# ddiazdom/grlBWT

Measured on AMD Instinct MI355X. Metric: input MB/s building BCR BWT on 10 GB DNA reads, 1/2/4/8 MI355X, higher is better.
Workload: dtype u8; 1 GPU; 66225166 x 150 bp Illumina-style reads (10000000066 bytes) from a 330000000 bp genome, 0.5% substitutions; BASELINE configs[3]; input_resident=HBM, output=.rl_bwt image in HBM, parallelism=1 GPU

## Files before the change

### grlbwt_amd/csrc/engine_impl.hpp

```cpp

#include "switches.hpp"

namespace GRL_NS {

using prim::u8;
using prim::u16;
using prim::u32;
using prim::u64;
typedef GRL_IDX_T idx_t;

template <class T>
struct DBuf {
    T *p = nullptr;
    u64 n = 0;
    DBuf() {}
    explicit DBuf(u64 n_) { alloc(n_); }
    DBuf(const DBuf &) = delete;
    DBuf &operator=(const DBuf &) = delete;
    DBuf(DBuf &&o) noexcept : p(o.p), n(o.n) { o.p = nullptr; o.n = 0; }
    DBuf &operator=(DBuf &&o) noexcept {
        if (this != &o) { release(); p = o.p; n = o.n; o.p = nullptr; o.n = 0; }
        return *this;
    }
    ~DBuf() { release(); }
    void alloc(u64 n_) { release(); p = (T *)prim::dev_alloc((n_ ? n_ : 1) * sizeof(T)); n = n_; }
    void release() { if (p) prim::dev_free(p); p = nullptr; n = 0; }
    void shrink(u64 n_) { if (p && n_ < n) { prim::dev_shrink(p, (n_ ? n_ : 1) * sizeof(T)); n = n_; } }
    void zero() { prim::dev_memset(p, 0, n * sizeof(T)); }
    void fill_ff() { prim::dev_memset(p, 0xFF, n * sizeof(T)); }
    std::vector<T> to_host(u64 cnt) const { std::vector<T> h(cnt); prim::d2h(h.data(), p, cnt * sizeof(T)); return h; }
    T get(u64 i) const { T v; prim::d2h(&v, p + i, sizeof(T)); return v; }
};

static inline unsigned bitlen64(u64 v) { return v == 0 ? 0 : 64 - (unsigned)__builtin_clzll(v); }

static inline bool test_fail_rank(int fail_rank, int me) {
    if constexpr (prim::kIsDevice) { (void)fail_rank; (void)me; return false; }
    else return fail_rank == me;
}

template <class T>
GRL_HD u64 upper_bound(const T *a, u64 n, T v) {
    u64 lo = 0, hi = n;
    while (lo < hi) { u64 mid = (lo + hi) >> 1; if (a[mid] <= v) lo = mid + 1; else hi = mid; }
// ... 639 lines not shown
    }
};
template <class F>
struct ListedFn {
    F f; const u64 *pos;
    static constexpr int kBatch = 1;
    static constexpr bool kClaims = F::kClaims;
    u64 *claim_bits = nullptr;
    GRL_DEV u64 claim_pos(u64 v) const { return pos[v]; }
    GRL_DEV bool is_start(u64) const { return true; }
    GRL_DEV u32 process(u64 v) const { return f.process(pos[v]); }
    GRL_DEV u32 operator()(u64 v) const { return f.process(pos[v]); }
    GRL_DEV void process_batch(const u64 *, const bool *, u32 *) const {}
    GRL_DEV void first_seen(u32 slot, u64 v) const { f.first_seen(slot, pos[v]); }
};

template <class cell_t, bool FIRST>
struct CompactTableFn {
    const cell_t *t;
    CellOps<cell_t, FIRST> ops;
    const u64 *startbits;
    const u64 *keys; const idx_t *counts;
    u64 *ph_pos; idx_t *ph_freq; u32 *ph_len; u32 *ph_slot; u8 *ph_lastT;
    int ks; u64 cs; const u64 *rep_pos;
    u64 n;
    GRL_DEV void emit(u64 s, u64 k) const {
        u64 k64 = keys[s << ks];
        u64 pos, len;
        bool lastT;
        if (k64 & kExactKey) {
// ... 43 lines not shown
        const u64 k0 = pbase[p], cnt = (u64)pbase[p + 1] - k0, src0 = pstart[p];
        for (u64 j = i & 63; j < cnt; j += 64) {
            const u64 k = k0 + j, src = src0 + j;
            const u64 hi = dhi[src];
            const prim::U128 r(rec_lo(dkey[src], hi), hi);
            const u32 f = dcnt[src];
            ph_key[k] = r; ph_pos[k] = 0; ph_freq[k] = (idx_t)f; ph_len[k] = rec_len(r); ph_slot[k] = slot0 + (u32)k;
            ph_lastT[k] = (r.hi & kPhrLastT) ? 1 : 0;
            ph_vflag[k] = (u8)((f > 1 ? 2u : 0u) | ((r.hi & kPhrLastT) ? 1u : 0u));
        }
    }
};
struct PartValFn {
    const u64 *pstart; const u32 *pbase; const u32 *lid; const u32 *slot_val; u32 slot0; u32 *out;
    const u8 *vflag;
    GRL_DEV void operator()(u64 i) const {
        const u64 p = i >> 6;
        const u64 a = pstart[p], e = pstart[p + 1], k0 = (u64)pbase[p], v0 = (u64)slot0 + k0;
        for (u64 x = a + (i & 63); x < e; x += 256) {
            u32 l[4], v[4];
#pragma unroll
            for (int j = 0; j < 4; j++) l[j] = x + 64u * j < e ? lid[x + 64u * j] : prim::kNoId;
#pragma unroll
            for (int j = 0; j < 4; j++) v[j] = l[j] == prim::kNoId ? 0u : (slot_val[v0 + (u64)l[j]] | (vflag ? (u32)vflag[k0 + (u64)l[j]] : 0u));
#pragma unroll
            for (int j = 0; j < 4; j++) if (x + 64u * j < e) out[x + 64u * j] = v[j];
        }
    }
};
struct PartCombineFn {
    const u32 *slot_val; const u32 *vals; u32 *text;
    GRL_DEV void operator()(u64 i) const { const u32 m = text[i]; text[i] = (m & kLongMark) ? slot_val[m & ~kLongMark] : vals[i]; }
};
struct LenIn {
    const u32 *l;
    GRL_DEV u32 operator()(u64 i) const { return l[i]; }
};
struct FreqLenIn {
    const idx_t *f; const u32 *l;
    GRL_DEV prim::Pair<u64, u64> operator()(u64 i) const { return prim::Pair<u64, u64>((u64)f[i], (u64)l[i]); }
};
GRL_HD u64 rank1(const u64 *words, const idx_t *base, u64 x);
template <class cell_t, bool FIRST, int PER = 4>
struct DictBuildFn {
    const cell_t *t;
    CellOps<cell_t, FIRST> ops;
    const u32 *ph_off; u64 D; u64 S; const u64 *ph_pos;
// ... 819 lines not shown
                u64 x = x16[k], w = x >> 6;
                if (w != cur) { prim::atomic_or(&words[cur * ws], m); m = 0; cur = w; }
                m |= 1ull << (x & 63);
            }
        }
        prim::atomic_or(&words[cur * ws], m);
    }
};
GRL_HD u64 rank1(const u64 *words, const idx_t *base, u64 x) {
    return (u64)base[x >> 6] + (u64)__builtin_popcountll(words[x >> 6] & ((1ull << (x & 63)) - 1ull));
}
static inline void build_rankbits(RankBits &rb, const idx_t *pos, u64 count, u64 nbits, const char *name) {
    u64 nw = nbits / 64 + 2;
    rb.words.alloc(nw);
    rb.base.alloc(nw + 1);
    rb.words.zero();
    prim::for_each((count + 15) / 16, BuildBitsFn{pos, count, rb.words.p}, name);
    prim::exclusive_scan_nosync<idx_t>(nw, PopcIn{rb.words.p}, rb.base.p, true, name);
}

struct BuildBits32Fn {
    const u32 *pos; u64 count; u64 *words;
    GRL_DEV void operator()(u64 j) const {
        u64 i0 = j * 16, i1 = i0 + 16 < count ? i0 + 16 : count;
        u64 cur = (u64)pos[i0] >> 6, m = 0;
        for (u64 i = i0; i < i1; i++) {
            u64 x = pos[i], w = x >> 6;
            if (w != cur) { prim::atomic_or(&words[cur], m); m = 0; cur = w; }
            m |= 1ull << (x & 63);
        }
        prim::atomic_or(&words[cur], m);
    }
};
static inline void build_rankbits32(RankBits &rb, const u32 *pos, u64 count, u64 nbits, const char *name) {
    u64 nw = nbits / 64 + 2;
    rb.words.alloc(nw);
    rb.base.alloc(nw + 1);
    rb.words.zero();
    prim::for_each((count + 15) / 16, BuildBits32Fn{pos, count, rb.words.p}, name);
    prim::exclusive_scan_nosync<idx_t>(nw, PopcIn{rb.words.p}, rb.base.p, true, name);
}

template <class L>
struct IdxIn {
    const L *p;
    GRL_DEV idx_t operator()(u64 i) const { return (idx_t)p[i]; }
};
struct SymHeadIn64 {
    const u32 *s;
    GRL_DEV u64 operator()(u64 t) const { return (t == 0 || s[t] != s[t - 1]) ? 1ull : 0ull; }
};
struct IdxIn64 {
    const idx_t *p;
// ... 1083 lines not shown
        prim::h2d(own0.p, host_cells, n * (u64)w);
        load_text(own0.p, n, w);
    }

    struct LocalParse {
        u64 n_occ = 0, D = 0, S = 0, cap = 0;
        u32 maxlen = 0;
        DBuf<u32> next_text;
        DBuf<u64> ph_pos; DBuf<idx_t> ph_freq; DBuf<u32> ph_len, ph_slot, ph_off; DBuf<u8> ph_lastT;
        u64 Ds = 0; int part_bits = 0, rec_b = 0; u32 slot0 = 0;
        DBuf<prim::U128> ph_key;
        DBuf<u32> lid, pbase;
        DBuf<u8> ph_vflag;
        DBuf<u64> pstart;
        prim::RecSort psort;
        void clear() {
            n_occ = D = S = cap = Ds = 0; maxlen = 0; part_bits = rec_b = 0; slot0 = 0;
            next_text.release(); ph_pos.release(); ph_freq.release(); ph_len.release(); ph_slot.release(); ph_off.release(); ph_lastT.release();
            ph_key.release(); ph_vflag.release(); pstart.release(); lid.release(); pbase.release(); psort.release();
        }
    };

    struct PartPlan { bool on = false; int rec_b = 0; u32 rec_cmax = 0; int part_bits = 0; };
    struct SamplePlan { u64 blk = 0, stride = 0, n = 0, distinct = 0, long_occ = 0; double frac = 1.0; };
    struct TablePlan { u64 cap = 0, cap_max = 0, cap_hot = 0; bool aggregate = false, interleaved = false, direct = false; int ks = 0; u64 cs = 1; u32 dir_b[3] = {0, 0, 0}; u64 sym_of_code = 0; };
    static bool direct_index_bits(const u64 sym_present[4], u32 bits[3], u64 &sym_of_code) {
        int syms[256], ns = 0;
        for (int i = 0; i < 256; i++) if ((sym_present[i >> 6] >> (i & 63)) & 1ull) syms[ns++] = i;
        if (ns > 8) return false;
        for (u32 a = 0; a < 8; a++) for (u32 b = a + 1; b < 8; b++) for (u32 c = b + 1; c < 8; c++) {
            u32 seen = 0; bool ok = true; u64 soc = 0;
            for (int k = 0; k < ns && ok; k++) {
// ... 41 lines not shown
            while (part.part_bits < 20 && (n_occ >> part.part_bits) > 5000) part.part_bits++;
            if (prim::sw().part_bits) part.part_bits = std::max(1, std::min(20, prim::sw().part_bits));
        }
        void sample_table() {
            tab.cap_max = 1024;
            while (tab.cap_max < 2 * n_occ && tab.cap_max < (1ull << 31)) tab.cap_max <<= 1;
            tab.cap = tab.cap_max;
            P.next_text.alloc(n_occ); scal.alloc(8); giant_list.alloc(giant_cap);
            StageTimer st(&E.tm.hash, "hash");
            const u64 want_s = (FIRST && n >= (1ull << 26)) ? (1ull << 22) : (1ull << 20), n_s = n < want_s ? n : want_s;
            if (n_s >= n) return;
            smp.blk = 4096; smp.stride = n / (n_s / smp.blk); smp.n = n_s;
            u64 cap_s = 1024; while (cap_s < 2 * n_s) cap_s <<= 1;
            DBuf<u64> tk(cap_s), trep; DBuf<idx_t> tc(cap_s);
            if (HF::kExact) trep.alloc(cap_s);
            tk.zero(); tc.zero(); scal.zero();
            HF fs{t, ops, startbits.p, wordbase.p, tk.p, cap_s - 1, cap_s, 0, P.next_text.p, scal.p, n, n_occ, trep.p};
            fs.rec_b = part.rec_b; fs.rec_cmax = part.rec_cmax;
            fs.walk_cap = HF::kLongWalk;
            prim::for_each_agg(n_s, SampledFn<HF>{fs, smp.blk, smp.stride}, SlotCountAdd{tc.p, 1}, true, "hash_sample");
            const prim::Pair<u64, u64> so = prim::reduce_sum<prim::Pair<u64, u64>>(cap_s, SampleCountIn{tk.p, tc.p}, "hash_sample_count");
            const u64 occ_s = std::max<u64>(so.b, 1);
            smp.distinct = so.a;
            if (part.on) smp.long_occ = occ_s;
            smp.frac = std::min(1.0, (double)smp.distinct / (double)occ_s);
            u64 want = (u64)(1.7 * smp.frac * (double)n_occ) + 4096;
            if (part.on) want = (u64)(3.0 * (double)smp.long_occ * ((double)n / (double)n_s)) + 4096;
            tab.cap = 4096; while (tab.cap < want) tab.cap <<= 1;
            if (tab.cap > tab.cap_max) tab.cap = tab.cap_max;
            if (prim::sw().table_trace) fprintf(stderr, "[grlbwt] level %d: sample %llu occurrences, %llu distinct -> table %llu slots for %llu occurrences\n",
                                                      prim::rt().tag, (unsigned long long)occ_s, (unsigned long long)smp.distinct, (unsigned long long)tab.cap, (unsigned long long)n_occ);
// ... 15 lines not shown
                }
            }
            const bool hot = !tab.direct && tab.aggregate && smp.n && !part.on && !prim::sw().no_hot_table;
            if (!tab.direct && !hot) return;
            if (tab.direct) tab.cap_hot = HF::kDirectSlots;
            else for (tab.cap_hot = 1024; tab.cap_hot < 4 * smp.distinct;) tab.cap_hot <<= 1;
            if (tab.cap_max > (1ull << 30)) tab.cap_max = 1ull << 30;
            if (tab.cap > tab.cap_max) tab.cap = tab.cap_max;
            if (!prim::sw().table_trace) return;
            if (tab.direct) fprintf(stderr, "[grlbwt] level %d: direct index on bits %u, %u, %u of a cell (%llu slots in front of the table)\n", prim::rt().tag,
                                    tab.dir_b[0], tab.dir_b[1], tab.dir_b[2], (unsigned long long)tab.cap_hot);
            else fprintf(stderr, "[grlbwt] level %d: hot table of %llu slots for the %llu phrases of the sample\n", prim::rt().tag,
                         (unsigned long long)tab.cap_hot, (unsigned long long)smp.distinct);
        }
        void alloc_table() {
            if (tab.interleaved) { keys.alloc(2 * tab.cap); keys.zero(); }
            else { keys.alloc(tab.cap_hot + tab.cap); counts.alloc(tab.cap_hot + tab.cap); keys.zero(); counts.zero(); }
            cnt = tab.interleaved ? (idx_t *)(keys.p + 1) : counts.p;
            if (HF::kExact) rep_pos.alloc(tab.cap_hot + tab.cap);
            scal.zero(); claim.zero();
        }
        void fill_hot_table(HF &f) {
            HF fh{t, ops, startbits.p, wordbase.p, keys.p, tab.cap_hot - 1, tab.cap_hot, 0, P.next_text.p, scal.p, n, n_occ, rep_pos.p, claim.p};
            fh.walk_cap = HF::kLongWalk;
            prim::for_each_agg(smp.n, SampledFn<HF>{fh, smp.blk, smp.stride, claim.p}, NoCountAdd{}, false, "hash_hot");
            f.hot_keys = keys.p; f.hot_mask = tab.cap_hot - 1; f.slot_base = (u32)tab.cap_hot;
        }
        void hash_listed(const HF &f, DBuf<u64> &lbits, bool aggregate) {
            DBuf<u32> lbase(nwords + 1);
            const u64 nl = (u64)prim::exclusive_scan<u32>(nwords, PopcIn32{lbits.p}, lbase.p, false, "hash_long_list");
            DBuf<u64> lpos(nl ? nl : 1);
            if (nl) prim::for_each(nwords, BitPositionsFn{lbits.p, lbase.p, lpos.p}, "hash_long_list");
            lbits.release(); lbase.release();
            if (nl) prim::for_each_agg(nl, ListedFn<HF>{f, lpos.p, claim.p}, SlotCountAdd{cnt, tab.cs}, aggregate, "hash_long_phrases");
        }
        void records_and_long_phrases(const HF &f) {
            prim::dev_memset(P.next_text.p, 0, n_occ * sizeof(u32));
            DBuf<u64> lbits(nwords + 1); lbits.zero();
            auto records = [&](auto bw) {
                prim::for_each_set_bit<idx_t>(n, startbits.p, wordbase.p, PhraseRecordFn<cell_t, decltype(bw)::value>{t, ops, startbits.p, wordbase.p, n, n_occ,
                                                                                                               rec_k.p, rec_hi.p, part.rec_b, part.rec_cmax, lbits.p, scal.p}, "hash_phrases");
            };
            switch (part.rec_b) {
#define GRL_REC_CASE(BW) case BW: records(std::integral_constant<int, BW>()); break;
                GRL_REC_CASE(10) GRL_REC_CASE(11) GRL_REC_CASE(12) GRL_REC_CASE(13) GRL_REC_CASE(14) GRL_REC_CASE(15) GRL_REC_CASE(16)
                GRL_REC_CASE(17) GRL_REC_CASE(18) GRL_REC_CASE(19) GRL_REC_CASE(20) GRL_REC_CASE(21) GRL_REC_CASE(22) GRL_REC_CASE(23)
                GRL_REC_CASE(24) GRL_REC_CASE(25) GRL_REC_CASE(26) GRL_REC_CASE(27) GRL_REC_CASE(28) GRL_REC_CASE(29) GRL_REC_CASE(30)
#undef GRL_REC_CASE
                default: records(std::integral_constant<int, 0>()); break;
            }
            hash_listed(f, lbits, false);
        }
        void name_stream_and_long_phrases(const HF &f) {
            DBuf<u64> lbits(nwords + 1); lbits.zero();
            prim::name_stream(n, f, SlotCountAdd{cnt, tab.cs}, lbits.p, "hash_phrases");
            hash_listed(f, lbits, tab.aggregate);
        }
        bool hash_pass() {
            alloc_table();
            HF f{t, ops, startbits.p, wordbase.p, keys.p + tab.cap_hot, tab.cap - 1, (tab.cap == tab.cap_max) ? tab.cap : 96 , tab.ks,
                 P.next_text.p, scal.p, n, n_occ, rep_pos.p ? rep_pos.p + tab.cap_hot : nullptr, claim.p};
            if (part.on) { f.rec_k = rec_k.p; f.rec_hi = rec_hi.p; f.rec_b = part.rec_b; f.rec_cmax = part.rec_cmax; }
            f.giant_list = giant_list.p; f.giant_n = scal.p + 4; f.giant_cap = (u32)std::min<u64>(giant_cap, 0xFFFFFFFFull);
            if (tab.direct) { f.dir_on = 1; f.dir_b0 = tab.dir_b[0]; f.dir_b1 = tab.dir_b[1]; f.dir_b2 = tab.dir_b[2]; f.dir_rep = rep_pos.p; f.slot_base = (u32)tab.cap_hot; }
            else if (tab.cap_hot) fill_hot_table(f);
            if constexpr (!FIRST) {
                if (part.on && !prim::sw().part_one_pass) records_and_long_phrases(f);
                else prim::for_each_agg(n, f, SlotCountAdd{cnt, tab.cs}, tab.aggregate, "hash_phrases");
            } else if (tab.direct && n_occ < 0xFFFFFFF0ull && !prim::sw().no_name_stream) name_stream_and_long_phrases(f);
// ... 421 lines not shown
        }
        void suffix_sort_local() {
            StageTimer st(&E.tm.dict_sort, "dict_sort");
            const u64 S = I.S, D = I.D, maxlen = I.maxlen;
            const u64 run_min = prim::sw().run_keys_min;
            RunKeys rk;
            DBuf<u32> run_rem, run_skip;
            const bool longmode = !C && (u64)maxlen >= run_min && S > 0;
            const u64 dbl_after = prim::sw().doubling_after;
            const SortKeyShape ks = sort_key_shape(I.sigma, I.maxlen, (maxlen >= run_min && S > 0) ? 1 + (int)bitlen64(maxlen) : 0);
            const int K = ks.K, b = ks.b;
            rk.rb = ks.rb;
            if (rk.rb) {
                DBuf<u32> rex(S), ends(S);
                run_rem.alloc(S); run_skip.alloc(S);
                run_skip.zero();
                prim::exclusive_scan_emit<u32>(S, RunChangeIn{dict_sym.p, pbits.words.p, S}, RunEndsEmitFn{rex.p, ends.p}, "suffix_runs");
                prim::for_each(S, RunRemFn{rex.p, ends.p, run_rem.p}, "suffix_runs");
                rk.rem = run_rem.p; rk.skip = run_skip.p;
            }
            const u32 cap = (u32)prim::sw().seg_cap;
            DBuf<u64> ka;
            {
                const SufKeep keep{dict_phr.p, I.ph_off, I.ph_lastT, longmode};
                if (!C) {
                    DBuf<u32> dropcnt(D + 1);
                    const u64 dropped = prim::exclusive_scan<u32>(D, PhraseDropIn{I.ph_off, I.ph_lastT, longmode}, dropcnt.p, true, "suffix_keep");
                    Sg = S - dropped;
                    ka.alloc(Sg); perm.alloc(Sg);
                    prim::for_each(S, Key0KeepFn{keep, dropcnt.p, dict_sym.p, K, b, ka.p, perm.p, rk}, "suffix_keys0");
                } else {
// ... 39 lines not shown
            u64 Lres = (u64)K, iters = 1;
            DBuf<u32> act;
            u64 A = Sg;
            bool refined = false, doubling = false;
            u64 Ld = 0, dbl_rounds = 0;
            DBuf<u32> slot_of, rank_ex, nskip;
            DBuf<u8> ures;
            for (;;) {
                SplitScan<u32, ByteIn> unres(A, ByteIn{uflag.p}, "suffix_unresolved_scan");
                const u64 U = unres.total;
                if (U == 0) break;
                if (Lres > (u64)maxlen + (u64)K || dbl_rounds > 80) throw prim::Error(-71, "suffix refinement does not terminate");
                if (!doubling && longmode && iters > dbl_after) {
                    doubling = true;
                    Ld = Lres;
                    if (!rk.rb) { run_skip.alloc(S); run_skip.zero(); rk.skip = run_skip.p; }
                    slot_of.alloc(S); slot_of.fill_ff();
                    prim::for_each(Sg, SlotOfFn{perm.p, slot_of.p}, "suffix_doubling");
                    ures.alloc(Sg); ures.zero();
                    prim::for_each(A, UresInitFn{refined ? act.p : nullptr, uflag.p, ures.p}, "suffix_doubling");
                    rank_ex.alloc(Sg + 1);
                }
                DBuf<u32> uslot(U), uq(U), hex(U + 1);
                DBuf<u64> ukey(U);
                DBuf<u8> uhead(U), unext(U);
                const UnresolvedItem compact{refined ? act.p : nullptr, perm.p, hflag.p, uslot.p, uq.p, uhead.p};
                if (doubling) {
                    prim::exclusive_scan_nosync<u32>(Sg, ByteIn{hflag.p}, rank_ex.p, false, "suffix_doubling");
                    nskip.alloc(U);
                    const DoubleKeyFn keys{compact, hflag.p, dict_phr.p, I.ph_off, slot_of.p, rank_ex.p, ures.p, rk.skip, Ld, Sg, ukey.p, nskip.p};
                    unres.emit(keys, "suffix_doubling");
                    dbl_rounds++;
                } else {
                    const ExtKeyFn keys{compact, dict_sym.p, pbits.words.p, S, Lres, K, b, ukey.p, rk};
// ... 338 lines not shown
        else if (Z.sharded) Z.suffix_sort_sharded();
        else { try { Z.suffix_sort_local(); } catch (const prim::Error &e) { C->fail(e); } }
        {
            StageTimer st(&tm.dict_groups, "dict_groups");
            if (Z.sharded && !Z.carry) Z.fetch_records();
            if (!C) Z.group_fold();
            else C->local([&] { Z.group_fold(); });
            Z.group_counts();
            Z.prebwt();
            Z.grammar();
            Z.phrase_values(phrase_val);
        }
        L.info.M = Z.M;
    }

    void emit_local(LocalParse &P, const u32 *val_of_local_phrase, DBuf<u32> *slot_val_filled = nullptr, bool rank_only = false) {
        StageTimer st(&tm.emit, "emit");
        DBuf<u32> own;
        if (!slot_val_filled) {
            own.alloc(P.cap);
            prim::for_each(P.D, ScatterValFn{P.ph_slot.p, val_of_local_phrase, own.p}, "slot_values");
        }
        const u32 *sv = slot_val_filled ? slot_val_filled->p : own.p;
        if (P.Ds || P.part_bits) {
            DBuf<u32> va(P.n_occ), vb(P.n_occ), vc(P.n_occ);
            prim::for_each(((u64)1 << P.part_bits) * 64, PartValFn{P.pstart.p, P.pbase.p, P.lid.p, sv, P.slot0, va.p, rank_only ? P.ph_vflag.p : nullptr}, "emit_part.values");
            P.pstart.release();
            P.psort.backward(va.p, vb.p, vc.p, "emit_part.back");
            prim::for_each(P.n_occ, PartCombineFn{sv, vc.p, P.next_text.p}, "emit_parse");
            P.psort.release(); P.lid.release(); P.pbase.release(); P.ph_key.release(); P.ph_vflag.release();
        } else prim::for_each((P.n_occ + 3) / 4, MapFn{sv, P.next_text.p, P.n_occ}, "emit_parse");
    }

    void finish_round(LocalParse &P, LevelData &L, u64 n_strings_for_termination, u64 n_occ_for_termination) {
        if (keep_texts) {
            DBuf<u32> cp(P.n_occ);
            prim::d2d(cp.p, P.next_text.p, P.n_occ * sizeof(u32));
            prim::sync();
            kept_texts.push_back(std::move(cp));
        }
        cur_text = std::move(P.next_text);
        cur_n = P.n_occ;
        cur_sigma = L.M;
        levels.push_back(std::move(L));
// ... 72 lines not shown
        if (B.D != stats.n_strings || !(cur_text.get(cur_n - 1) & 1u)) throw prim::Error(-71, "base case: the level's text does not hold one flagged cell per string");
        B.maxlen = prim::reduce_max<u32>(B.D, OffLenIn{B.off.p}, "base_maxlen");
        return B;
    }
    bool base_case_candidate() const {
        const u64 ratio = prim::sw().base_case_ratio;
        if (ratio == 0 || keep_texts || parse_done || levels.size() < 2) return false;
        if (cur_n >= 0xFFFFFFF0ull || stats.n_strings >= 0xFFFFFFF0ull) return false;
        return cur_n / ratio < stats.n_strings || (cur_n / ratio == stats.n_strings && cur_n % ratio == 0);
    }
    void base_bwt(BaseText &B) {
        prim::rt().tag = (int)levels.size();
        prim::rt().phase = 'i';
        const u64 n = cur_n, D = B.D;
        DBuf<u8> all_last(D);
        all_last.fill_ff();
        DictIn<u32, false> I;
        I.D = D; I.S = n; I.maxlen = B.maxlen; I.sigma = cur_sigma;
        I.ph_off = B.off.p; I.ph_lastT = all_last.p;
        LevelData scratch;
        DictStage<u32, false> Z(*this, I, scratch);
        Z.want_groups = false;
        Z.dict_sym = std::move(B.sym); Z.dict_phr = std::move(B.str);
        {
            StageTimer st(&tm.ind_assemble, "ind_assemble");
            build_rankbits32(Z.pbits, I.ph_off, D, n + 1, "base_text");
        }
        Z.suffix_sort_local();
        if (Z.Sg != n) throw prim::Error(-71, "base case: the sort left suffixes out");
        StageTimer st(&tm.ind_assemble, "ind_assemble");
        DBuf<u32> s(n);
// ... 209 lines not shown
    struct AsmIn { const u32 *psym; const idx_t *plen; u64 P; const u32 *u_to_p; const u32 *p_to_u; u64 M; u32 sigma; u64 n_out; };
    struct AsmStage {
        Engine &eng; const AsmIn &L; LevelInfo &I; const CellView cells; const u64 E, Tsum; const int r; const bool to_image; const LevelCodes code; const u64 R;
        DBuf<u32> esym; DBuf<idx_t> epos; u64 Re = 0;
        DBuf<RankCell> tstarts;
        u64 NH = 0, G = 0;
        DBuf<idx_t> nh_len; DBuf<u32> nh_sym; DBuf<RankCell> kinds;
        Runs out; u64 Ro = 0;
        AsmStage(Engine &e, const AsmIn &l, LevelInfo &i, u32 u0, u64 tsum, int r_, bool img) : eng(e), L(l), I(i), cells(e.cells.view(u0)), E(e.cells.E), Tsum(tsum),
            r(r_), to_image(img), code(l.sigma), R(e.bwt.R) {}
        void truns(DBuf<idx_t> &Tpos, DBuf<u32> &term) {
            esym.alloc(R ? R : 1); epos.alloc(R + 1);
            Re = R ? (u64)prim::exclusive_scan_emit<idx_t>(R, TermHeadIn{term.p}, TermHeadEmitFn{term.p, Tpos.p, esym.p, epos.p}, "asm.truns") : 0;
            Tpos.release(); term.release(); eng.bwt.sym.release(); eng.bwt.len.release();
            const u64 nwT = Tsum / 64 + 2;
            tstarts.alloc(nwT); tstarts.zero();
            if (Re) prim::for_each((Re + 15) / 16, BuildBitsFn{epos.p, Re, reinterpret_cast<u64 *>(tstarts.p), 2}, "asm.tbits");
            prim::exclusive_scan_emit_nosync<u64>(nwT, RankCellPopcIn{tstarts.p}, RankCellBaseEmitFn{tstarts.p}, "asm.tbits");
        }
        void place_prebwt() {
            const u64 P = L.P, M = L.M;
            DBuf<idx_t> nhb(P + 1);
            NH = (u64)prim::exclusive_scan<idx_t>(P, NotCodeIn{L.psym, code.hocc}, nhb.p, true, "asm.nhb");
            I.G = G = NH + E;
            DBuf<idx_t> seg_pos(NH ? NH : 1);
            nh_len.alloc(NH ? NH : 1); nh_sym.alloc(NH ? NH : 1);
            {
                DBuf<idx_t> first_cell;
                if (P * 32 > E && L.p_to_u) {
                    first_cell.alloc(M + 1);
                    DBuf<idx_t> bstart1(M), bend(M);
                    bstart1.zero(); bend.zero();
                    prim::for_each(E, BucketEdgesFn{cells, E, bstart1.p, bend.p}, "asm.first_cell");
                    prim::exclusive_scan_nosync<idx_t>(M, BucketSizeIn{bstart1.p, bend.p}, first_cell.p, true, "asm.first_cell");
                }
                prim::for_each(P, PrePlaceFn{L.psym, L.plen, nhb.p, L.u_to_p, M, cells, E, L.p_to_u, first_cell.p, code.hocc,
                                             seg_pos.p, nh_sym.p, nh_len.p}, "asm.pre_place");
            }
            nhb.release();
            const u64 nwG = G / 64 + 2;
            kinds.alloc(nwG); kinds.zero();
            if (NH) prim::for_each((NH + 15) / 16, BuildBitsFn{seg_pos.p, NH, reinterpret_cast<u64 *>(kinds.p), 2}, "asm.kinds");
            prim::exclusive_scan_emit_nosync<u64>(nwG, RankCellPopcIn{kinds.p}, RankCellBaseEmitFn{kinds.p}, "asm.kinds");
        }
        typedef prim::SmPlan<idx_t> Plan;
        struct PlanGuard { Plan &p; ~PlanGuard() { p.release(); } };
        void check_totals(const Plan &plan) const {
            if (plan.take_total != Tsum) throw prim::Error(-71, "induction: BWT_{r+1} consumption mismatch (level " + std::to_string(r) + ": " +
                                                                    std::to_string(plan.take_total) + " vs " + std::to_string(Tsum) + ")");
            if (plan.len_total != L.n_out) throw prim::Error(-71, "induction: BWT of level " + std::to_string(r) + " describes " + std::to_string(plan.len_total) +
                                                                      " symbols, the level has " + std::to_string(L.n_out));
        }
        bool one_walk(const AsmSeg &seg, Plan &plan, bool mostly_plain) {
            if (prim::sw().asm_two_pass || (mostly_plain && !prim::sw().asm_one_walk)) return false;
            const u64 cap = G + Re + 1;
            const u64 qcap = Re / prim::kSmInline + 1;
// ... 747 lines not shown
```

### grlbwt_amd/csrc/prim_hip.hpp

```cpp
#pragma once
#include <hip/hip_runtime.h>
#include <cstdint>
#include <cstdio>
#include <cstdlib>
#include <cstring>
#include <chrono>
#include <stdexcept>
#include <string>
#include <vector>
#include <map>
#include <utility>
#include <type_traits>

#define GRLBWT_PRIM_HIP 1
#include "switches.hpp"

#define GRL_HD __host__ __device__ __forceinline__
#define GRL_DEV __device__ __forceinline__

namespace prim {

typedef uint8_t u8;
typedef uint16_t u16;
typedef uint32_t u32;
// ... 460 lines not shown
inline void pinned_free(void *p) { if (p) (void)hipHostFree(p); }
inline void h2d_async(void *d, const void *h, size_t n) { if (n) GRL_HIP_CHECK(hipMemcpyAsync(d, h, n, hipMemcpyHostToDevice, rt().stream)); }
inline void d2h_async(void *h, const void *d, size_t n) { if (n) GRL_HIP_CHECK(hipMemcpyAsync(h, d, n, hipMemcpyDeviceToHost, rt().stream)); }
struct Fence { hipEvent_t e = nullptr; bool armed = false; };
inline void fence_record(Fence &f) {
    if (!f.e) GRL_HIP_CHECK(hipEventCreateWithFlags(&f.e, hipEventDisableTiming));
    GRL_HIP_CHECK(hipEventRecord(f.e, rt().stream));
    f.armed = true;
}
inline void fence_wait(Fence &f) { if (f.armed) { GRL_HIP_CHECK(hipEventSynchronize(f.e)); f.armed = false; } }
inline void thread_attach() { if (rt().device >= 0) (void)hipSetDevice(rt().device); }
inline void fence_destroy(Fence &f) { if (f.e) (void)hipEventDestroy(f.e); f.e = nullptr; f.armed = false; }
inline void d2d(void *dst, const void *src, size_t n) {
    if (n) GRL_HIP_CHECK(hipMemcpyAsync(dst, src, n, hipMemcpyDeviceToDevice, rt().stream));
}
inline void dev_memset(void *d, int v, size_t n) {
    if (n) GRL_HIP_CHECK(hipMemsetAsync(d, v, n, rt().stream));
}

GRL_DEV u32 atomic_add(u32 *p, u32 v) { return atomicAdd(p, v); }
GRL_DEV u64 atomic_add(u64 *p, u64 v) {
    return (u64)atomicAdd(reinterpret_cast<unsigned long long *>(p), (unsigned long long)v);
}
GRL_DEV void atomic_or(u64 *p, u64 v) {
    atomicOr(reinterpret_cast<unsigned long long *>(p), (unsigned long long)v);
}
GRL_DEV u32 atomic_min(u32 *p, u32 v) { return atomicMin(p, v); }
GRL_DEV u32 atomic_max(u32 *p, u32 v) { return atomicMax(p, v); }
GRL_DEV u64 atomic_min(u64 *p, u64 v) { return (u64)atomicMin(reinterpret_cast<unsigned long long *>(p), (unsigned long long)v); }
GRL_DEV u64 atomic_max(u64 *p, u64 v) { return (u64)atomicMax(reinterpret_cast<unsigned long long *>(p), (unsigned long long)v); }
GRL_DEV u64 atomic_cas(u64 *p, u64 expect, u64 desired) {
    return (u64)atomicCAS(reinterpret_cast<unsigned long long *>(p), (unsigned long long)expect,
// ... 2423 lines not shown
}
inline int sort_keys_fwd(u32 *a, u32 *b, u64 n, int begin_bit, int end_bit, const char *name) {
    return sort_keys<u32, 1>(a, b, n, begin_bit, end_bit, name);
}


struct alignas(16) U128 {
    u64 lo, hi;
    U128() = default;
    GRL_HD U128(int) : lo(0), hi(0) {}
    GRL_HD U128(u64 l, u64 h) : lo(l), hi(h) {}
    GRL_HD bool operator==(const U128 &o) const { return lo == o.lo && hi == o.hi; }
};
static constexpr u32 kNoId = 0xFFFFFFFFu;

template <class W, int DB, int TB>
__global__ void __launch_bounds__(TB)
    k_rs_unscatter(const u16 *rank_in, const W *src, W *dst, u64 n, const u64 *offsets , u32 tiles) {
    constexpr int NB = 1 << DB, TILE = TB * kRsItems, NW = TB / 64;
    static_assert(NB <= TB, "one thread per digit");
    __shared__ u16 s_d[TILE];
    __shared__ W s_v[TILE];
    __shared__ u64 s_gbase[NB];
    __shared__ u32 s_wsum[NW];
    const int lane = threadIdx.x & 63, w = threadIdx.x >> 6;
    const u32 tile = blockIdx.x;
    const u64 base = (u64)tile * TILE;
    const u64 left = n - base;
    const u32 tile_n = left < (u64)TILE ? (u32)left : (u32)TILE;
    u16 rk[kRsItems];
#pragma unroll
    for (int j = 0; j < kRsItems; j++) { const u32 t = (u32)j * TB + threadIdx.x; rk[j] = t < tile_n ? rank_in[base + t] : (u16)0; }
    for (u32 t = threadIdx.x; t < (u32)TILE; t += TB) s_d[t] = 0;
// ... 38 lines not shown
        if (lane == 0) before = 0;
        for (int k = 0; k < w; k++) before = s_wsum[k] > before ? s_wsum[k] : before;
#pragma unroll
        for (int j = 0; j < kRsItems; j++) s_d[t0 + j] = (u16)(dloc[j] > before ? dloc[j] : before);
    }
    __syncthreads();
#pragma unroll
    for (int j = 0; j < kRsItems; j++) {
        const u32 t = (u32)j * TB + threadIdx.x;
        if (t < tile_n) s_v[t] = src[s_gbase[s_d[t]] + t];
    }
    __syncthreads();
#pragma unroll
    for (int j = 0; j < kRsItems; j++) {
        const u32 t = (u32)j * TB + threadIdx.x;
        if (t < tile_n) dst[base + t] = s_v[rk[j]];
    }
}

struct RecSort {
    u64 n = 0;
    int bits = 0, passes = 0, shifts[4] = {0, 0, 0, 0}, widths[4] = {0, 0, 0, 0};
    u32 tiles = 0;
    u16 *rnk[4] = {nullptr, nullptr, nullptr, nullptr};
    u64 *offs[4] = {nullptr, nullptr, nullptr, nullptr};
    static constexpr int kThreads = 1024;
    GRL_HD static u64 part_of(u64 key, int bits_) { return bits_ ? (key * kMixMul) >> (64 - bits_) : 0; }
    int forward(u64 *key_a, u64 *hi_a, u64 *key_b, u64 *hi_b, u64 n_, int bits_, const char *name = "rec_sort") {
        release();
        n = n_; bits = bits_;
        if (n == 0 || bits <= 0) { bits = 0; return 0; }
        if (bits > 27) throw Error(-22, "RecSort: more than 2^27 partitions");
        passes = (bits + 8) / 9;
// ... 11 lines not shown
        int cur = 0;
        for (int p = 0; p < passes; p++) {
            const int db = widths[p] <= 8 ? 8 : 9;
            rnk[p] = (u16 *)dev_alloc(n * sizeof(u16));
            offs[p] = (u64 *)dev_alloc(((u64)1 << db) * tiles * sizeof(u64));
            const u32 dmask = (1u << widths[p]) - 1u;
            u64 *kin = cur ? key_b : key_a, *kout = cur ? key_a : key_b, *vin = cur ? hi_b : hi_a, *vout = cur ? hi_a : hi_b;
            if (db == 8) rs_pass<u64, u64, 2, 8, kThreads, true>(kin, vin, kout, vout, n, shifts[p], dmask, tiles, counts, offs[p], chunk_sums, chunk_off, name, rnk[p]);
            else rs_pass<u64, u64, 2, 9, kThreads, true>(kin, vin, kout, vout, n, shifts[p], dmask, tiles, counts, offs[p], chunk_sums, chunk_off, name, rnk[p]);
            cur ^= 1;
        }
        dev_free(counts); dev_free(chunk_sums); dev_free(chunk_off);
        return cur;
    }
    template <class W>
    void backward(W *in, W *tmp, W *out, const char *name = "rec_sort.back") const {
        if (n == 0) return;
        if (passes == 0) { d2d(out, in, n * sizeof(W)); return; }
        W *src = in;
        for (int p = passes - 1; p >= 0; p--) {
            W *dst = (p == 0) ? out : ((src == tmp) ? in : tmp);
            prof_begin(name, n * (sizeof(u16) + 2 * sizeof(W)));
            if (widths[p] <= 8) hipLaunchKernelGGL((k_rs_unscatter<W, 8, kThreads>), dim3(tiles), dim3(kThreads), 0, rt().stream, (const u16 *)rnk[p], src, dst, n, offs[p], tiles);
            else hipLaunchKernelGGL((k_rs_unscatter<W, 9, kThreads>), dim3(tiles), dim3(kThreads), 0, rt().stream, (const u16 *)rnk[p], src, dst, n, offs[p], tiles);
            prof_end();
            after_launch(name);
            src = dst;
        }
    }
    void release() {
        for (int p = 0; p < 4; p++) {
            if (rnk[p]) dev_free(rnk[p]);
            if (offs[p]) dev_free(offs[p]);
            rnk[p] = nullptr; offs[p] = nullptr;
        }
        passes = 0; n = 0; bits = 0;
    }
    RecSort() {}
    RecSort(const RecSort &) = delete;
// ... 1017 lines not shown
        }
    }
}

inline int ac_table_bits() {
    const int b = sw().alpha_table_bits;
    return b < 2 ? 2 : (b > 26 ? 26 : b);
}
template <class cell_t>
inline void ac_collect(const cell_t *t, u64 n, AcPlan &P) {
    P.release();
    P.bits = ac_table_bits();
    const u64 cap = (u64)1 << P.bits;
    P.tab = (u64 *)dev_alloc(cap * 16);
    P.scal = (u32 *)dev_alloc(16);
    dev_memset(P.tab, 0xFF, cap * 16);
    dev_memset(P.scal, 0, 16);
    prof_begin("alpha.collect", n * sizeof(cell_t));
    hipLaunchKernelGGL((k_ac_collect<cell_t>), dim3(grid_for(n, kBlock)), dim3(kBlock), 0, rt().stream, t, n, P.tab, P.bits, (u32)(cap / 2), P.scal);
    prof_end();
    after_launch("alpha.collect");
    u32 h[2];
    d2h(h, P.scal, 8);
    P.sigma = h[0];
    P.overflow = h[1] != 0;
}
template <class cell_t>
inline void ac_rank(const cell_t *t, u64 n, AcPlan &P, int key_bits, u64 *values, u32 *ranks) {
    const u64 cap = (u64)1 << P.bits, sigma = P.sigma;
    u64 *tmp = (u64 *)dev_alloc((sigma ? sigma : 1) * 8);
    dev_memset(P.scal, 0, 16);
// ... 395 lines not shown
```

Measured before the change: 16400 MB/s.

## Write listed long-phrase values once and skip sentinels in partition unscatter

When long phrases are few, their occurrence ordinals are recorded and their values are written directly into the next-level text. The final radix unscatter then skips sentinel entries instead of producing a full temporary array that a combine pass merges. This removes one n_occ-sized buffer, a full combine pass and the up-front memset of next_text, at the cost of an extra ordinal kernel and a conditional store in the unscatter. It also adds profiling labels on memsets.

```diff
diff --git a/grlbwt_amd/csrc/engine_impl.hpp b/grlbwt_amd/csrc/engine_impl.hpp
--- a/grlbwt_amd/csrc/engine_impl.hpp
+++ b/grlbwt_amd/csrc/engine_impl.hpp
@@ -26,8 +26,15 @@
     void alloc(u64 n_) { release(); p = (T *)prim::dev_alloc((n_ ? n_ : 1) * sizeof(T)); n = n_; }
     void release() { if (p) prim::dev_free(p); p = nullptr; n = 0; }
     void shrink(u64 n_) { if (p && n_ < n) { prim::dev_shrink(p, (n_ ? n_ : 1) * sizeof(T)); n = n_; } }
-    void zero() { prim::dev_memset(p, 0, n * sizeof(T)); }
-    void fill_ff() { prim::dev_memset(p, 0xFF, n * sizeof(T)); }
+    void fill(int v, const char *site) {
+#ifdef GRLBWT_PRIM_HIP
+        prim::dev_memset(p, v, n * sizeof(T), site);
+#else
+        (void)site; prim::dev_memset(p, v, n * sizeof(T));
+#endif
+    }
+    void zero(const char *site = nullptr) { fill(0, site); }
+    void fill_ff(const char *site = nullptr) { fill(0xFF, site); }
     std::vector<T> to_host(u64 cnt) const { std::vector<T> h(cnt); prim::d2h(h.data(), p, cnt * sizeof(T)); return h; }
     T get(u64 i) const { T v; prim::d2h(&v, p + i, sizeof(T)); return v; }
 };
@@ -697,6 +704,13 @@
     GRL_DEV void process_batch(const u64 *, const bool *, u32 *) const {}
     GRL_DEV void first_seen(u32 slot, u64 v) const { f.first_seen(slot, pos[v]); }
 };
+struct ListedOrdinalFn {
+    const u64 *pos; const u64 *startbits; const idx_t *wordbase; u32 *ord;
+    GRL_DEV void operator()(u64 v) const {
+        const u64 p = pos[v];
+        ord[v] = (u32)((u64)wordbase[p >> 6] + (u64)__builtin_popcountll(startbits[p >> 6] & ((1ull << (p & 63)) - 1ull)));
+    }
+};
 
 template <class cell_t, bool FIRST>
 struct CompactTableFn {
@@ -770,6 +784,7 @@
 struct PartValFn {
     const u64 *pstart; const u32 *pbase; const u32 *lid; const u32 *slot_val; u32 slot0; u32 *out;
     const u8 *vflag;
+    u32 none;
     GRL_DEV void operator()(u64 i) const {
         const u64 p = i >> 6;
         const u64 a = pstart[p], e = pstart[p + 1], k0 = (u64)pbase[p], v0 = (u64)slot0 + k0;
@@ -778,7 +793,7 @@
 #pragma unroll
             for (int j = 0; j < 4; j++) l[j] = x + 64u * j < e ? lid[x + 64u * j] : prim::kNoId;
 #pragma unroll
-            for (int j = 0; j < 4; j++) v[j] = l[j] == prim::kNoId ? 0u : (slot_val[v0 + (u64)l[j]] | (vflag ? (u32)vflag[k0 + (u64)l[j]] : 0u));
+            for (int j = 0; j < 4; j++) v[j] = l[j] == prim::kNoId ? none : (slot_val[v0 + (u64)l[j]] | (vflag ? (u32)vflag[k0 + (u64)l[j]] : 0u));
 #pragma unroll
             for (int j = 0; j < 4; j++) if (x + 64u * j < e) out[x + 64u * j] = v[j];
         }
@@ -787,6 +802,15 @@
 struct PartCombineFn {
     const u32 *slot_val; const u32 *vals; u32 *text;
     GRL_DEV void operator()(u64 i) const { const u32 m = text[i]; text[i] = (m & kLongMark) ? slot_val[m & ~kLongMark] : vals[i]; }
+};
+static constexpr u32 kNoVal = 0xFFFFFFFFu;
+struct LongValFn {
+    const u32 *lord; const u32 *slot_val; u32 *text;
+    GRL_DEV void operator()(u64 j) const {
+        const u64 o = (u64)lord[j];
+        const u32 m = text[o];
+        if (m & kLongMark) text[o] = slot_val[m & ~kLongMark];
+    }
 };
 struct LenIn {
     const u32 *l;
@@ -1636,7 +1660,7 @@
     u64 nw = nbits / 64 + 2;
     rb.words.alloc(nw);
     rb.base.alloc(nw + 1);
-    rb.words.zero();
+    rb.words.zero((std::string(name) + ".clear").c_str());
     prim::for_each((count + 15) / 16, BuildBitsFn{pos, count, rb.words.p}, name);
     prim::exclusive_scan_nosync<idx_t>(nw, PopcIn{rb.words.p}, rb.base.p, true, name);
 }
@@ -1658,7 +1682,7 @@
     u64 nw = nbits / 64 + 2;
     rb.words.alloc(nw);
     rb.base.alloc(nw + 1);
-    rb.words.zero();
+    rb.words.zero((std::string(name) + ".clear").c_str());
     prim::for_each((count + 15) / 16, BuildBits32Fn{pos, count, rb.words.p}, name);
     prim::exclusive_scan_nosync<idx_t>(nw, PopcIn{rb.words.p}, rb.base.p, true, name);
 }
@@ -2772,8 +2796,11 @@
         DBuf<u8> ph_vflag;
         DBuf<u64> pstart;
         prim::RecSort psort;
+        bool listed = false; u64 n_long = 0;
+        DBuf<u32> lord;
         void clear() {
             n_occ = D = S = cap = Ds = 0; maxlen = 0; part_bits = rec_b = 0; slot0 = 0;
+            listed = false; n_long = 0; lord.release();
             next_text.release(); ph_pos.release(); ph_freq.release(); ph_len.release(); ph_slot.release(); ph_off.release(); ph_lastT.release();
             ph_key.release(); ph_vflag.release(); pstart.release(); lid.release(); pbase.release(); psort.release();
         }
@@ -2845,7 +2872,7 @@
             u64 cap_s = 1024; while (cap_s < 2 * n_s) cap_s <<= 1;
             DBuf<u64> tk(cap_s), trep; DBuf<idx_t> tc(cap_s);
             if (HF::kExact) trep.alloc(cap_s);
-            tk.zero(); tc.zero(); scal.zero();
+            tk.zero("hash_sample.clear"); tc.zero("hash_sample.clear"); scal.zero();
             HF fs{t, ops, startbits.p, wordbase.p, tk.p, cap_s - 1, cap_s, 0, P.next_text.p, scal.p, n, n_occ, trep.p};
             fs.rec_b = part.rec_b; fs.rec_cmax = part.rec_cmax;
             fs.walk_cap = HF::kLongWalk;
@@ -2891,11 +2918,11 @@
                          (unsigned long long)tab.cap_hot, (unsigned long long)smp.distinct);
         }
         void alloc_table() {
-            if (tab.interleaved) { keys.alloc(2 * tab.cap); keys.zero(); }
-            else { keys.alloc(tab.cap_hot + tab.cap); counts.alloc(tab.cap_hot + tab.cap); keys.zero(); counts.zero(); }
+            if (tab.interleaved) { keys.alloc(2 * tab.cap); keys.zero("hash_table.clear"); }
+            else { keys.alloc(tab.cap_hot + tab.cap); counts.alloc(tab.cap_hot + tab.cap); keys.zero("hash_table.clear"); counts.zero("hash_table.clear"); }
             cnt = tab.interleaved ? (idx_t *)(keys.p + 1) : counts.p;
             if (HF::kExact) rep_pos.alloc(tab.cap_hot + tab.cap);
-            scal.zero(); claim.zero();
+            scal.zero(); claim.zero("hash_claims.clear");
         }
         void fill_hot_table(HF &f) {
             HF fh{t, ops, startbits.p, wordbase.p, keys.p, tab.cap_hot - 1, tab.cap_hot, 0, P.next_text.p, scal.p, n, n_occ, rep_pos.p, claim.p};
@@ -2903,17 +2930,22 @@
             prim::for_each_agg(smp.n, SampledFn<HF>{fh, smp.blk, smp.stride, claim.p}, NoCountAdd{}, false, "hash_hot");
             f.hot_keys = keys.p; f.hot_mask = tab.cap_hot - 1; f.slot_base = (u32)tab.cap_hot;
         }
-        void hash_listed(const HF &f, DBuf<u64> &lbits, bool aggregate) {
+        void hash_listed(const HF &f, DBuf<u64> &lbits, bool aggregate, bool keep_ordinals = false) {
             DBuf<u32> lbase(nwords + 1);
             const u64 nl = (u64)prim::exclusive_scan<u32>(nwords, PopcIn32{lbits.p}, lbase.p, false, "hash_long_list");
             DBuf<u64> lpos(nl ? nl : 1);
             if (nl) prim::for_each(nwords, BitPositionsFn{lbits.p, lbase.p, lpos.p}, "hash_long_list");
             lbits.release(); lbase.release();
+            const bool keep = keep_ordinals && n_occ <= 0xFFFFFFFFull && nl <= n_occ / 16;
+            P.listed = keep; P.n_long = keep ? nl : 0; P.lord.release();
+            if (keep_ordinals && !keep) P.next_text.zero("hash_phrases.clear");
             if (nl) prim::for_each_agg(nl, ListedFn<HF>{f, lpos.p, claim.p}, SlotCountAdd{cnt, tab.cs}, aggregate, "hash_long_phrases");
+            if (!keep) return;
+            P.lord.alloc(nl);
+            if (nl) prim::for_each(nl, ListedOrdinalFn{lpos.p, startbits.p, wordbase.p, P.lord.p}, "hash_long_list");
         }
         void records_and_long_phrases(const HF &f) {
-            prim::dev_memset(P.next_text.p, 0, n_occ * sizeof(u32));
-            DBuf<u64> lbits(nwords + 1); lbits.zero();
+            DBuf<u64> lbits(nwords + 1); lbits.zero("hash_phrases.clear");
             auto records = [&](auto bw) {
                 prim::for_each_set_bit<idx_t>(n, startbits.p, wordbase.p, PhraseRecordFn<cell_t, decltype(bw)::value>{t, ops, startbits.p, wordbase.p, n, n_occ,
                                                                                                                rec_k.p, rec_hi.p, part.rec_b, part.rec_cmax, lbits.p, scal.p}, "hash_phrases");
@@ -2926,10 +2958,10 @@
 #undef GRL_REC_CASE
                 default: records(std::integral_constant<int, 0>()); break;
             }
-            hash_listed(f, lbits, false);
+            hash_listed(f, lbits, false, true);
         }
         void name_stream_and_long_phrases(const HF &f) {
-            DBuf<u64> lbits(nwords + 1); lbits.zero();
+            DBuf<u64> lbits(nwords + 1); lbits.zero("hash_phrases.clear");
             prim::name_stream(n, f, SlotCountAdd{cnt, tab.cs}, lbits.p, "hash_phrases");
             hash_listed(f, lbits, tab.aggregate);
         }
@@ -3381,7 +3413,7 @@
             if (rk.rb) {
                 DBuf<u32> rex(S), ends(S);
                 run_rem.alloc(S); run_skip.alloc(S);
-                run_skip.zero();
+                run_skip.zero("suffix_runs.clear");
                 prim::exclusive_scan_emit<u32>(S, RunChangeIn{dict_sym.p, pbits.words.p, S}, RunEndsEmitFn{rex.p, ends.p}, "suffix_runs");
                 prim::for_each(S, RunRemFn{rex.p, ends.p, run_rem.p}, "suffix_runs");
                 rk.rem = run_rem.p; rk.skip = run_skip.p;
@@ -3451,10 +3483,10 @@
                 if (!doubling && longmode && iters > dbl_after) {
                     doubling = true;
                     Ld = Lres;
-                    if (!rk.rb) { run_skip.alloc(S); run_skip.zero(); rk.skip = run_skip.p; }
-                    slot_of.alloc(S); slot_of.fill_ff();
+                    if (!rk.rb) { run_skip.alloc(S); run_skip.zero("suffix_doubling.clear"); rk.skip = run_skip.p; }
+                    slot_of.alloc(S); slot_of.fill_ff("suffix_doubling.clear");
                     prim::for_each(Sg, SlotOfFn{perm.p, slot_of.p}, "suffix_doubling");
-                    ures.alloc(Sg); ures.zero();
+                    ures.alloc(Sg); ures.zero("suffix_doubling.clear");
                     prim::for_each(A, UresInitFn{refined ? act.p : nullptr, uflag.p, ures.p}, "suffix_doubling");
                     rank_ex.alloc(Sg + 1);
                 }
@@ -3823,6 +3855,19 @@
         L.info.M = Z.M;
     }
 
+    struct CopyValFn {
+        const u32 *v; u32 *text;
+        GRL_DEV void operator()(u64 i) const { const u32 x = v[i]; if (x != kNoVal) text[i] = x; }
+    };
+    static void back_unless_none(const prim::RecSort &psort, DBuf<u32> &va, DBuf<u32> &vb, DBuf<u32> &text) {
+#ifdef GRLBWT_PRIM_HIP
+        psort.backward_skip(va.p, vb.p, text.p, kNoVal, "emit_part.back");
+#else
+        DBuf<u32> vc(text.n);
+        psort.backward(va.p, vb.p, vc.p, "emit_part.back");
+        prim::for_each(text.n, CopyValFn{vc.p, text.p}, "emit_part.back");
+#endif
+    }
     void emit_local(LocalParse &P, const u32 *val_of_local_phrase, DBuf<u32> *slot_val_filled = nullptr, bool rank_only = false) {
         StageTimer st(&tm.emit, "emit");
         DBuf<u32> own;
@@ -3832,11 +3877,22 @@
         }
         const u32 *sv = slot_val_filled ? slot_val_filled->p : own.p;
         if (P.Ds || P.part_bits) {
-            DBuf<u32> va(P.n_occ), vb(P.n_occ), vc(P.n_occ);
-            prim::for_each(((u64)1 << P.part_bits) * 64, PartValFn{P.pstart.p, P.pbase.p, P.lid.p, sv, P.slot0, va.p, rank_only ? P.ph_vflag.p : nullptr}, "emit_part.values");
+            DBuf<u32> va(P.n_occ), vb(P.n_occ), vc;
+            prim::for_each(((u64)1 << P.part_bits) * 64, PartValFn{P.pstart.p, P.pbase.p, P.lid.p, sv, P.slot0, va.p, rank_only ? P.ph_vflag.p : nullptr,
+                                                                   P.listed ? kNoVal : 0u}, "emit_part.values");
             P.pstart.release();
-            P.psort.backward(va.p, vb.p, vc.p, "emit_part.back");
-            prim::for_each(P.n_occ, PartCombineFn{sv, vc.p, P.next_text.p}, "emit_parse");
+            if (prim::sw().table_trace) fprintf(stderr, "[grlbwt] level %d: parse from the partitions: %llu occurrences, %llu record phrases, %llu table phrases, %llu listed occurrences (%s)\n",
+                                                      prim::rt().tag, (unsigned long long)P.n_occ, (unsigned long long)P.Ds, (unsigned long long)(P.D - P.Ds),
+                                                      (unsigned long long)P.n_long, P.listed ? "written once" : "combined");
+            if (P.listed) {
+                if (P.n_long) prim::for_each(P.n_long, LongValFn{P.lord.p, sv, P.next_text.p}, "emit_parse.long");
+                P.lord.release();
+                back_unless_none(P.psort, va, vb, P.next_text);
+            } else {
+                vc.alloc(P.n_occ);
+                P.psort.backward(va.p, vb.p, vc.p, "emit_part.back");
+                prim::for_each(P.n_occ, PartCombineFn{sv, vc.p, P.next_text.p}, "emit_parse");
+            }
             P.psort.release(); P.lid.release(); P.pbase.release(); P.ph_key.release(); P.ph_vflag.release();
         } else prim::for_each((P.n_occ + 3) / 4, MapFn{sv, P.next_text.p, P.n_occ}, "emit_parse");
     }
@@ -3939,7 +3995,7 @@
         prim::rt().phase = 'i';
         const u64 n = cur_n, D = B.D;
         DBuf<u8> all_last(D);
-        all_last.fill_ff();
+        all_last.fill_ff("base_bwt.clear");
         DictIn<u32, false> I;
         I.D = D; I.S = n; I.maxlen = B.maxlen; I.sigma = cur_sigma;
         I.ph_off = B.off.p; I.ph_lastT = all_last.p;
@@ -4179,7 +4235,7 @@
             Re = R ? (u64)prim::exclusive_scan_emit<idx_t>(R, TermHeadIn{term.p}, TermHeadEmitFn{term.p, Tpos.p, esym.p, epos.p}, "asm.truns") : 0;
             Tpos.release(); term.release(); eng.bwt.sym.release(); eng.bwt.len.release();
             const u64 nwT = Tsum / 64 + 2;
-            tstarts.alloc(nwT); tstarts.zero();
+            tstarts.alloc(nwT); tstarts.zero("asm.tbits.clear");
             if (Re) prim::for_each((Re + 15) / 16, BuildBitsFn{epos.p, Re, reinterpret_cast<u64 *>(tstarts.p), 2}, "asm.tbits");
             prim::exclusive_scan_emit_nosync<u64>(nwT, RankCellPopcIn{tstarts.p}, RankCellBaseEmitFn{tstarts.p}, "asm.tbits");
         }
@@ -4195,7 +4251,7 @@
                 if (P * 32 > E && L.p_to_u) {
                     first_cell.alloc(M + 1);
                     DBuf<idx_t> bstart1(M), bend(M);
-                    bstart1.zero(); bend.zero();
+                    bstart1.zero("asm.first_cell.clear"); bend.zero("asm.first_cell.clear");
                     prim::for_each(E, BucketEdgesFn{cells, E, bstart1.p, bend.p}, "asm.first_cell");
                     prim::exclusive_scan_nosync<idx_t>(M, BucketSizeIn{bstart1.p, bend.p}, first_cell.p, true, "asm.first_cell");
                 }
@@ -4204,7 +4260,7 @@
             }
             nhb.release();
             const u64 nwG = G / 64 + 2;
-            kinds.alloc(nwG); kinds.zero();
+            kinds.alloc(nwG); kinds.zero("asm.kinds.clear");
             if (NH) prim::for_each((NH + 15) / 16, BuildBitsFn{seg_pos.p, NH, reinterpret_cast<u64 *>(kinds.p), 2}, "asm.kinds");
             prim::exclusive_scan_emit_nosync<u64>(nwG, RankCellPopcIn{kinds.p}, RankCellBaseEmitFn{kinds.p}, "asm.kinds");
         }
diff --git a/grlbwt_amd/csrc/prim_hip.hpp b/grlbwt_amd/csrc/prim_hip.hpp
--- a/grlbwt_amd/csrc/prim_hip.hpp
+++ b/grlbwt_amd/csrc/prim_hip.hpp
@@ -498,8 +498,11 @@
 inline void d2d(void *dst, const void *src, size_t n) {
     if (n) GRL_HIP_CHECK(hipMemcpyAsync(dst, src, n, hipMemcpyDeviceToDevice, rt().stream));
 }
-inline void dev_memset(void *d, int v, size_t n) {
-    if (n) GRL_HIP_CHECK(hipMemsetAsync(d, v, n, rt().stream));
+inline void dev_memset(void *d, int v, size_t n, const char *site = nullptr) {
+    if (!n) return;
+    if (site) prof_begin(site, n);
+    GRL_HIP_CHECK(hipMemsetAsync(d, v, n, rt().stream));
+    if (site) prof_end();
 }
 
 GRL_DEV u32 atomic_add(u32 *p, u32 v) { return atomicAdd(p, v); }
@@ -2953,9 +2956,9 @@
 };
 static constexpr u32 kNoId = 0xFFFFFFFFu;
 
-template <class W, int DB, int TB>
+template <class W, int DB, int TB, bool SKIP = false>
 __global__ void __launch_bounds__(TB)
-    k_rs_unscatter(const u16 *rank_in, const W *src, W *dst, u64 n, const u64 *offsets , u32 tiles) {
+    k_rs_unscatter(const u16 *rank_in, const W *src, W *dst, u64 n, const u64 *offsets , u32 tiles, W skip) {
     constexpr int NB = 1 << DB, TILE = TB * kRsItems, NW = TB / 64;
     static_assert(NB <= TB, "one thread per digit");
     __shared__ u16 s_d[TILE];
@@ -3024,9 +3027,17 @@
 #pragma unroll
     for (int j = 0; j < kRsItems; j++) {
         const u32 t = (u32)j * TB + threadIdx.x;
-        if (t < tile_n) dst[base + t] = s_v[rk[j]];
-    }
-}
+        if (t < tile_n) {
+            const W v = s_v[rk[j]];
+            if (!SKIP || !(v == skip)) dst[base + t] = v;
+        }
+    }
+}
+template <class W>
+struct CopyUnlessFn {
+    const W *src; W *dst; W skip;
+    GRL_DEV void operator()(u64 i) const { const W v = src[i]; if (!(v == skip)) dst[i] = v; }
+};
 
 struct RecSort {
     u64 n = 0;
@@ -3068,15 +3079,28 @@
         return cur;
     }
     template <class W>
-    void backward(W *in, W *tmp, W *out, const char *name = "rec_sort.back") const {
+    void backward(W *in, W *tmp, W *out, const char *name = "rec_sort.back") const { backward_as<W, false>(in, tmp, out, W(), name); }
+    template <class W>
+    void backward_skip(W *in, W *tmp, W *out, W skip, const char *name = "rec_sort.back") const { backward_as<W, true>(in, tmp, out, skip, name); }
+    template <class W, bool SKIP>
+    void backward_as(W *in, W *tmp, W *out, W skip, const char *name) const {
         if (n == 0) return;
-        if (passes == 0) { d2d(out, in, n * sizeof(W)); return; }
+        if (passes == 0) {
+            if (SKIP) for_each(n, CopyUnlessFn<W>{in, out, skip}, name);
+            else d2d(out, in, n * sizeof(W));
+            return;
+        }
         W *src = in;
         for (int p = passes - 1; p >= 0; p--) {
             W *dst = (p == 0) ? out : ((src == tmp) ? in : tmp);
             prof_begin(name, n * (sizeof(u16) + 2 * sizeof(W)));
-            if (widths[p] <= 8) hipLaunchKernelGGL((k_rs_unscatter<W, 8, kThreads>), dim3(tiles), dim3(kThreads), 0, rt().stream, (const u16 *)rnk[p], src, dst, n, offs[p], tiles);
-            else hipLaunchKernelGGL((k_rs_unscatter<W, 9, kThreads>), dim3(tiles), dim3(kThreads), 0, rt().stream, (const u16 *)rnk[p], src, dst, n, offs[p], tiles);
+            if (SKIP && p == 0) {
+                if (widths[p] <= 8) hipLaunchKernelGGL((k_rs_unscatter<W, 8, kThreads, SKIP>), dim3(tiles), dim3(kThreads), 0, rt().stream, (const u16 *)rnk[p], (const W *)src, dst, n, (const u64 *)offs[p], tiles, skip);
+                else hipLaunchKernelGGL((k_rs_unscatter<W, 9, kThreads, SKIP>), dim3(tiles), dim3(kThreads), 0, rt().stream, (const u16 *)rnk[p], (const W *)src, dst, n, (const u64 *)offs[p], tiles, skip);
+            } else {
+                if (widths[p] <= 8) hipLaunchKernelGGL((k_rs_unscatter<W, 8, kThreads, false>), dim3(tiles), dim3(kThreads), 0, rt().stream, (const u16 *)rnk[p], (const W *)src, dst, n, (const u64 *)offs[p], tiles, skip);
+                else hipLaunchKernelGGL((k_rs_unscatter<W, 9, kThreads, false>), dim3(tiles), dim3(kThreads), 0, rt().stream, (const u16 *)rnk[p], (const W *)src, dst, n, (const u64 *)offs[p], tiles, skip);
+            }
             prof_end();
             after_launch(name);
             src = dst;
@@ -4124,7 +4148,7 @@
     const u64 cap = (u64)1 << P.bits;
     P.tab = (u64 *)dev_alloc(cap * 16);
     P.scal = (u32 *)dev_alloc(16);
-    dev_memset(P.tab, 0xFF, cap * 16);
+    dev_memset(P.tab, 0xFF, cap * 16, "alpha.collect.clear");
     dev_memset(P.scal, 0, 16);
     prof_begin("alpha.collect", n * sizeof(cell_t));
     hipLaunchKernelGGL((k_ac_collect<cell_t>), dim3(grid_for(n, kBlock)), dim3(kBlock), 0, rt().stream, t, n, P.tab, P.bits, (u32)(cap / 2), P.scal);
```

Result: no change. 16550 MB/s (median of 6 runs) (+1.0%).
